# POSTECH-CVLab/RoDyGS

Measured on AMD Instinct MI355X. Metric: train-step fps at 1M dynamic Gaussians / 1080p (fwd+bwd+Adam, one camera per GPU per step), higher is better.
Workload: dtype f32; 1 GPU; 1000000 dynamic Gaussians + deformation MLP, 1920x1080, SH3, 100-frame synthetic video (BASELINE configs[2]); points=1000000, width=1920, height=1080, scene=uniform, frames=100, deferred_overflow_check=True, frame_order=orbit positions, bit-reversed, one_device=False, graph_replay=False, densify_stats=True, deterministic_backward=True, render_normal=True, parallelism=single GPU (frame-dp1), losses=photometric, sh_adam_in_backward=True, binning=bucket

## Files before the change

### rodygs_amd/csrc/rdg_render.hip

```cpp
#include "rdg_common.h"

#define RDG_BATCH 256

__device__ __forceinline__ int rdg_tile_of_block(int bid, int n_tiles) {
    const int per = (n_tiles + 7) >> 3;
    return (bid & 7) * per + (bid >> 3);
}

__device__ __forceinline__ float rdg_edge_min(float a, float b2, float c, float inv_c, float ue, float v0, float v1) {
    const float t = b2 * ue;
    const float vs = __builtin_amdgcn_fmed3f(-0.5f * t * inv_c, v0, v1);
    return fmaf(fmaf(c, vs, t), vs, a * ue * ue);
}
__device__ __forceinline__ uint32_t rdg_quadrant_bits(const float4 q0, const float4 q1, const float inv_cyy, float X0, float Y0) {
    const float a = q0.z, b = q0.w, o = q1.y;
    const float c = (b * b) / a + inv_cyy;
    const float t255 = 255.0f * o;
    if (!(t255 >= 0.99f)) return 0u;
    const float det = a * c - b * b;
    if (!(det > 0.0f) || !(a > 0.0f) || !(c > 0.0f)) return 0u;
    const float r2 = 2.0f * (__logf(t255) + 0.02f) * 1.001f;
    const float inv_a = 1.0f / a, inv_c = 1.0f / c, b2 = 2.0f * b;
    uint32_t bits = 0u;
#pragma unroll
    for (int qy = 0; qy < 2; ++qy) {
        const float v1 = q0.y - (Y0 + 8.0f * qy), v0 = v1 - 7.0f;
#pragma unroll
        for (int qx = 0; qx < 2; ++qx) {
            const float u1 = q0.x - (X0 + 8.0f * qx), u0 = u1 - 7.0f;
            const bool inside = u0 <= 0.0f && u1 >= 0.0f && v0 <= 0.0f && v1 >= 0.0f;
            const float m = fminf(fminf(rdg_edge_min(a, b2, c, inv_c, u0, v0, v1), rdg_edge_min(a, b2, c, inv_c, u1, v0, v1)),
                                  fminf(rdg_edge_min(c, b2, a, inv_a, v0, u0, u1), rdg_edge_min(c, b2, a, inv_a, v1, u0, u1)));
            bits |= (uint32_t)(inside || !(m > r2)) << (qy * 2 + qx);
        }
    }
    return bits;
}

#define RDG_NEG_LOG2E (-1.4426950408889634f)
struct RdgConicS { float hA, beta, gam; };
__device__ __forceinline__ RdgConicS rdg_stage_conic(float a, float b, float inv_cyy) {
    const float A2 = RDG_NEG_LOG2E * a, B = RDG_NEG_LOG2E * b;
    RdgConicS s;
    s.hA = 0.5f * A2;
    s.beta = (A2 < 0.0f) ? B / A2 : 0.0f;
    s.gam = (0.5f * RDG_NEG_LOG2E) * inv_cyy;
    return s;
}
__device__ __forceinline__ float rdg_log2_gauss(float hA, float beta, float gam, float dx, float dy) {
    const float w = fmaf(beta, dy, dx);
    return fmaf(hA * w, w, (gam * dy) * dy);
}
__device__ __forceinline__ float rdg_log2_gauss_w(float hA, float beta, float gam, float dx, float dy, float& w) {
    w = fmaf(beta, dy, dx);
    return fmaf(hA * w, w, (gam * dy) * dy);
}

__device__ __forceinline__ bool rdg_any(bool p) { return __builtin_amdgcn_ballot_w64(p) != 0ull; }
__device__ __forceinline__ bool rdg_all(bool p) { return __builtin_amdgcn_ballot_w64(!p) == 0ull; }

__device__ __forceinline__ unsigned long long rdg_uniform_u64(unsigned long long v) {
    const uint32_t lo = __builtin_amdgcn_readfirstlane((uint32_t)v);
    const uint32_t hi = __builtin_amdgcn_readfirstlane((uint32_t)(v >> 32));
    return ((unsigned long long)hi << 32) | lo;
}

#define RDG_THR_LIVE (0x80000000u | 0x3b808081u)
#define RDG_THR_DONE 0xffffffffu
template <bool NORMAL, bool CAPPED>
__device__ __forceinline__ void rdg_fwd_walk(unsigned long long mask, const unsigned long long cap, const int sbase,
                                             const uint32_t wbase, const char* sQ0, const char* sQ1, const char* sQ2,
                                             const char* sQ3, const float pixx, const float pixy,
                                             unsigned long long& seen, uint32_t& thrU, float& T,
                                             uint32_t& last_contributor, float& C0, float& C1, float& C2, float& Dp,
                                             float& N0, float& N1, float& N2) {
    while (mask) {
        const int jb = __builtin_ctzll(mask);
        asm("s_bitset0_b64 %0, %1" : "+s"(mask) : "s"(jb));
        int aj = (jb << 4) + sbase;
        asm volatile("" : "+v"(aj));
#ifdef RDG_ABL_FXSALU
        asm volatile("s_add_u32 s90, s90, 1\n\ts_add_u32 s91, s91, 1\n\ts_add_u32 s90, s90, 1\n\ts_add_u32 s91, s91, 1\n\t"
                     "s_add_u32 s90, s90, 1\n\ts_add_u32 s91, s91, 1\n\ts_add_u32 s90, s90, 1\n\ts_add_u32 s91, s91, 1" ::: "s90", "s91", "scc");
#endif
#ifdef RDG_ABL_FXVALU
        { float xa = T, xb = C0;
          asm volatile("v_mov_b32 %0, %1\n\tv_mov_b32 %1, %0\n\tv_mov_b32 %0, %1\n\tv_mov_b32 %1, %0\n\t"
                       "v_mov_b32 %0, %1\n\tv_mov_b32 %1, %0\n\tv_mov_b32 %0, %1\n\tv_mov_b32 %1, %0" : "+v"(xa), "+v"(xb)); }
#endif
        const float4 q0 = *(const float4*)(sQ0 + aj);
        const float2 q1 = *(const float2*)(sQ1 + aj);
        const float dx = q0.x - pixx, dy = q0.y - pixy;
        const float power = rdg_log2_gauss(q0.z, q0.w, q1.x, dx, dy);
        float alpha = q1.y * __builtin_amdgcn_exp2f(power);
        if (CAPPED && ((cap >> jb) & 1ull)) {
            asm volatile("; opacity above the cap" ::: "memory");
            alpha = fminf(RDG_ALPHA_CAP, alpha);
        }
        const uint32_t key = (__float_as_uint(power) & 0x80000000u) | __float_as_uint(alpha);
        const unsigned long long cand = __builtin_amdgcn_ballot_w64(key >= thrU);
        if (!cand) continue;
        asm("s_bitset1_b64 %0, %1" : "+s"(seen) : "s"(jb));
        float aeff;
        asm("v_cndmask_b32_e64 %0, 0, %1, %2" : "=v"(aeff) : "v"(alpha), "s"(cand));
        float test_T = T * (1.0f - aeff);
        float wgt = aeff * T;
        const float4 q2 = *(const float4*)(sQ2 + aj);
        const uint32_t idx = wbase + (uint32_t)jb;
        unsigned long long upd = cand;
        const unsigned long long stopm = __builtin_amdgcn_ballot_w64(test_T < RDG_T_STOP);
        if (stopm) {
            const bool stop = test_T < RDG_T_STOP;
            upd &= ~stopm;
            wgt = stop ? 0.0f : wgt;
            test_T = stop ? T : test_T;
            thrU = stop ? RDG_THR_DONE : thrU;
            if (rdg_all(thrU == RDG_THR_DONE)) { mask = 0ull; }
        }
        T = test_T;
        asm volatile("s_mov_b64 exec, %1\n\tv_mov_b32 %0, %2\n\ts_mov_b64 exec, -1"
                     : "+v"(last_contributor) : "s"(upd), "s"(idx));
        C0 += wgt * q2.x; C1 += wgt * q2.y; C2 += wgt * q2.z;
        Dp += wgt * q2.w;
        if (NORMAL) {
            const float4 q3 = *(const float4*)(sQ3 + aj);
            N0 += wgt * q3.x; N1 += wgt * q3.y; N2 += wgt * q3.z;
        }
    }
}


template <bool NORMAL>
__device__ __forceinline__ void
rdg_fwd_composite(const int k_begin, const int k_end, const uint2 range, const float X0, const float Y0, const float pixx,
                  const float pixy, const uint32_t* __restrict__ point_list, const RdgRec* __restrict__ rec,
                  unsigned long long* __restrict__ hit, float4* sQ0, float4* sQ1, float4* sQ2, float4* sQ3,
                  unsigned long long (*sMask)[4], unsigned long long* sCap, uint32_t& thrU, float& T, float& C0, float& C1,
                  float& C2, float& Dp, float& N0, float& N1, float& N2, uint32_t& last_contributor) {
    const int tid = threadIdx.x;
    const int lane = tid & 63, wv = tid >> 6;
    const int rounds = (k_end - k_begin + RDG_BATCH - 1) / RDG_BATCH;
    for (int r = 0; r < rounds; ++r) {
        if (__syncthreads_count(thrU == RDG_THR_DONE) == 256) break;
        const int k = k_begin + r * RDG_BATCH + tid;
        uint32_t qbits = 0;
        bool over_cap = false;
        if (k < k_end) {
            const uint32_t id = point_list[range.x + k];
            const RdgRec* p = rec + id;
            const float4 q0 = p->q0, q1 = p->q1, q2 = p->q2;
            const RdgConicS cs = rdg_stage_conic(q0.z, q0.w, q2.w);
            sQ0[tid] = make_float4(q0.x, q0.y, cs.hA, cs.beta);
            *(float2*)&sQ1[tid] = make_float2(cs.gam, q1.y);
            sQ2[tid] = make_float4(q2.x, q2.y, q2.z, q1.z);
            if (NORMAL) sQ3[tid] = p->q3;
            qbits = rdg_quadrant_bits(q0, q1, q2.w, X0, Y0);
            over_cap = q1.y > RDG_ALPHA_CAP;
        }
#pragma unroll
        for (int q = 0; q < 4; ++q) {
            const unsigned long long m = __ballot((qbits >> q) & 1u);
            if (lane == 0) sMask[q][wv] = m;
        }
        {
            const unsigned long long m = __ballot(over_cap);
            if (lane == 0) sCap[wv] = m;
        }
        __syncthreads();
#pragma unroll 1
        for (int s = 0; s < 4; ++s) {
            if (rdg_all(thrU == RDG_THR_DONE)) break;
            const unsigned long long mask = rdg_uniform_u64(sMask[wv][s]);
            const unsigned long long cap = rdg_uniform_u64(sCap[s]);
            unsigned long long seen = 0ull;
            const uint32_t wbase = (uint32_t)(k_begin + r * RDG_BATCH + s * 64 + 1);
            if (cap)
                rdg_fwd_walk<NORMAL, true>(mask, cap, s * 1024, wbase, (const char*)sQ0, (const char*)sQ1, (const char*)sQ2,
                                           (const char*)sQ3, pixx, pixy, seen, thrU, T, last_contributor, C0, C1, C2, Dp,
                                           N0, N1, N2);
            else
                rdg_fwd_walk<NORMAL, false>(mask, cap, s * 1024, wbase, (const char*)sQ0, (const char*)sQ1, (const char*)sQ2,
                                            (const char*)sQ3, pixx, pixy, seen, thrU, T, last_contributor, C0, C1, C2, Dp,
                                            N0, N1, N2);
            if (lane == 0 && seen) hit[(size_t)((k_begin >> 6) + r * 4 + s) * 4 + wv] = seen;
        }
    }
}

template <bool NORMAL>
__global__ void __launch_bounds__(256)
rdg_render_fwd_kernel(int W, int H, int gx, int n_tiles, const float* __restrict__ bg,
                      const uint2* __restrict__ ranges, const uint32_t* __restrict__ point_list,
                      const RdgRec* __restrict__ rec, long long capacity, const int32_t* __restrict__ num_rendered,
                      float* __restrict__ final_T, uint32_t* __restrict__ n_contrib, float* __restrict__ out_color,
                      float* __restrict__ out_depth, float* __restrict__ out_normal, float* __restrict__ out_alpha,
                      unsigned long long* __restrict__ hitbits, int split_min, uint4* __restrict__ zero_buf,
                      long long zero_n16) {
    if (zero_buf) {
        const long long per = (zero_n16 + gridDim.x - 1) / gridDim.x;
        const long long z0 = per * blockIdx.x, z1 = z0 + per < zero_n16 ? z0 + per : zero_n16;
        for (long long i = z0 + threadIdx.x; i < z1; i += 256) zero_buf[i] = make_uint4(0u, 0u, 0u, 0u);
    }
    const int tile = rdg_tile_of_block(blockIdx.x, n_tiles);
    if (tile >= n_tiles) return;
    __shared__ float4 sQ0[RDG_BATCH], sQ1[RDG_BATCH], sQ2[RDG_BATCH], sQ3[RDG_BATCH];
    __shared__ unsigned long long sMask[4][4];
    __shared__ unsigned long long sCap[4];
#ifdef RDG_ABL_FPAD
    __shared__ float sPad[RDG_ABL_FPAD];
    if (W < 0) sPad[threadIdx.x] = 1.0f;
#endif
    const int tid = threadIdx.x;
    const int lane = tid & 63, wv = tid >> 6;
    const int tx = tile % gx, ty = tile / gx;
    const int pxi = tx * RDG_TILE + (wv & 1) * 8 + (lane & 7);
    const int pyi = ty * RDG_TILE + (wv >> 1) * 8 + (lane >> 3);
    const bool inside = pxi < W && pyi < H;
    float pixx = (float)pxi, pixy = (float)pyi;
    asm volatile("" : "+v"(pixx), "+v"(pixy));
    const float X0 = (float)(tx * RDG_TILE), Y0 = (float)(ty * RDG_TILE);
    const uint2 range = ranges[tile];
    const int todo_total = (int)(range.y - range.x);
    if (todo_total > split_min) return;
    unsigned long long* const hit = hitbits + ((size_t)(range.x >> 6) + (size_t)tile) * 4;

    uint32_t thrU = inside ? RDG_THR_LIVE : RDG_THR_DONE;
    float T = 1.0f;
    float C0 = 0.f, C1 = 0.f, C2 = 0.f, Dp = 0.f, N0 = 0.f, N1 = 0.f, N2 = 0.f;
    uint32_t last_contributor = 0;
    rdg_fwd_composite<NORMAL>(0, todo_total, range, X0, Y0, pixx, pixy, point_list, rec, hit, sQ0, sQ1, sQ2, sQ3, sMask,
                              sCap, thrU, T, C0, C1, C2, Dp, N0, N1, N2, last_contributor);
    if (inside) {
        const size_t hw = (size_t)H * W;
        const size_t pid = (size_t)pyi * W + pxi;
        final_T[pid] = T;
        n_contrib[pid] = last_contributor;
        out_color[pid] = C0 + T * bg[0];
        out_color[hw + pid] = C1 + T * bg[1];
        out_color[2 * hw + pid] = C2 + T * bg[2];
        out_depth[pid] = Dp;
        out_alpha[pid] = 1.0f - T;
        out_normal[pid] = N0; out_normal[hw + pid] = N1; out_normal[2 * hw + pid] = N2;
    }
}

#define RDG_SEG_TS 0
#define RDG_SEG_TOUT 1
#define RDG_SEG_C 2
#define RDG_SEG_LAST 9
#define RDG_SEG_LIVE 10

__device__ __forceinline__ float* rdg_seg_row(float* seg_pix, uint32_t seg, int field) {
    return seg_pix + ((size_t)seg * RDG_SEG_F + field) * RDG_TILE_PIX;
}

__global__ void __launch_bounds__(256)
rdg_render_seg_T_kernel(int W, int H, int gx, const uint2* __restrict__ ranges, const uint32_t* __restrict__ point_list,
                        const RdgRec* __restrict__ rec, const uint32_t* __restrict__ sp_header,
                        const uint4* __restrict__ sp_work, float* __restrict__ seg_pix) {
    __shared__ float4 sQ0[RDG_BATCH];
    __shared__ float2 sQ1[RDG_BATCH];
    const int tid = threadIdx.x;
    const uint32_t n_work = sp_header[0];
    for (uint32_t wi = blockIdx.x; wi < n_work; wi += gridDim.x) {
        const uint4 w = sp_work[wi];
        const int tile = (int)w.x;
        const int tx = tile % gx, ty = tile / gx;
        const int wv = tid >> 6, lane = tid & 63;
        const int pxi = tx * RDG_TILE + (wv & 1) * 8 + (lane & 7);
        const int pyi = ty * RDG_TILE + (wv >> 1) * 8 + (lane >> 3);
        const float pixx = (float)pxi, pixy = (float)pyi;
        const uint2 range = ranges[tile];
        const int k_begin = (int)w.y * RDG_SPLIT_SEG, k_end = min(k_begin + RDG_SPLIT_SEG, (int)(range.y - range.x));
        float T = 1.0f;
        for (int k0 = k_begin; k0 < k_end; k0 += RDG_BATCH) {
            __syncthreads();
            const int k = k0 + tid;
            if (k < k_end) {
                const RdgRec* p = rec + point_list[range.x + k];
                const float4 q0 = p->q0, q1 = p->q1;
                const RdgConicS cs = rdg_stage_conic(q0.z, q0.w, p->q2.w);
                sQ0[tid] = make_float4(q0.x, q0.y, cs.hA, cs.beta);
                sQ1[tid] = make_float2(cs.gam, q1.y);
            }
            __syncthreads();
            const int n = min(RDG_BATCH, k_end - k0);
            for (int j = 0; j < n; ++j) {
                const float4 q0 = sQ0[j];
                const float2 q1 = sQ1[j];
                const float dx = q0.x - pixx, dy = q0.y - pixy;
                const float power = rdg_log2_gauss(q0.z, q0.w, q1.x, dx, dy);
                float alpha = q1.y * __builtin_amdgcn_exp2f(power);
                if (q1.y > RDG_ALPHA_CAP) alpha = fminf(RDG_ALPHA_CAP, alpha);
                const uint32_t key = (__float_as_uint(power) & 0x80000000u) | __float_as_uint(alpha);
                if (key >= RDG_THR_LIVE) T = T * (1.0f - alpha);
            }
        }
        rdg_seg_row(seg_pix, w.w + w.y, RDG_SEG_TS)[tid] = T;
    }
}

template <bool NORMAL>
__global__ void __launch_bounds__(256)
rdg_render_seg_kernel(int W, int H, int gx, const uint2* __restrict__ ranges, const uint32_t* __restrict__ point_list,
                      const RdgRec* __restrict__ rec, const uint32_t* __restrict__ sp_header,
                      const uint4* __restrict__ sp_work, float* __restrict__ seg_pix,
                      unsigned long long* __restrict__ hitbits) {
    __shared__ float4 sQ0[RDG_BATCH], sQ1[RDG_BATCH], sQ2[RDG_BATCH], sQ3[RDG_BATCH];
    __shared__ unsigned long long sMask[4][4];
    __shared__ unsigned long long sCap[4];
    const int tid = threadIdx.x;
    const int lane = tid & 63, wv = tid >> 6;
    const uint32_t n_work = sp_header[0];
    for (uint32_t wi = blockIdx.x; wi < n_work; wi += gridDim.x) {
// ... 54 lines not shown
        float T = 1.0f, C0 = 0.f, C1 = 0.f, C2 = 0.f, Dp = 0.f, N0 = 0.f, N1 = 0.f, N2 = 0.f;
        uint32_t last = 0;
        for (uint32_t s = 0; s < t.y; ++s) {
            const float* base = seg_pix + (size_t)(t.z + s) * RDG_SEG_F * RDG_TILE_PIX + tid;
            if (base[RDG_SEG_LIVE * RDG_TILE_PIX] == 0.0f) continue;
            T = base[RDG_SEG_TOUT * RDG_TILE_PIX];
            C0 += base[(RDG_SEG_C + 0) * RDG_TILE_PIX]; C1 += base[(RDG_SEG_C + 1) * RDG_TILE_PIX];
            C2 += base[(RDG_SEG_C + 2) * RDG_TILE_PIX]; Dp += base[(RDG_SEG_C + 3) * RDG_TILE_PIX];
            if (NORMAL) {
                N0 += base[(RDG_SEG_C + 4) * RDG_TILE_PIX]; N1 += base[(RDG_SEG_C + 5) * RDG_TILE_PIX];
                N2 += base[(RDG_SEG_C + 6) * RDG_TILE_PIX];
            }
            last = max(last, __float_as_uint(base[RDG_SEG_LAST * RDG_TILE_PIX]));
        }
        const size_t hw = (size_t)H * W;
        const size_t pid = (size_t)pyi * W + pxi;
        final_T[pid] = T;
        n_contrib[pid] = last;
        out_color[pid] = C0 + T * bg[0];
        out_color[hw + pid] = C1 + T * bg[1];
        out_color[2 * hw + pid] = C2 + T * bg[2];
        out_depth[pid] = Dp;
        out_alpha[pid] = 1.0f - T;
        out_normal[pid] = N0; out_normal[hw + pid] = N1; out_normal[2 * hw + pid] = N2;
    }
}

__global__ void __launch_bounds__(1024)
rdg_split_build_kernel(int n_tiles, const uint2* __restrict__ ranges, long long capacity,
                       const int32_t* __restrict__ num_rendered, uint32_t* __restrict__ sp_header,
                       uint4* __restrict__ sp_work, uint4* __restrict__ sp_tiles, uint32_t max_seg, uint32_t max_tiles) {
    __shared__ uint32_t sSeg, sTiles;
    if (threadIdx.x == 0) { sSeg = 0u; sTiles = 0u; }
    __syncthreads();
    if ((long long)num_rendered[0] <= capacity)
        for (int i = threadIdx.x; i < n_tiles; i += 1024) {
            const uint2 r = ranges[i];
            const uint32_t n = r.y - r.x;
            if (n > (uint32_t)RDG_SPLIT_MIN) {
                const uint32_t nseg = (n + RDG_SPLIT_SEG - 1) / RDG_SPLIT_SEG;
                const uint32_t base = atomicAdd(&sSeg, nseg), ti = atomicAdd(&sTiles, 1u);
                if (base + nseg <= max_seg && ti < max_tiles) {
                    sp_tiles[ti] = make_uint4((uint32_t)i, nseg, base, 0u);
                    for (uint32_t c = 0; c < nseg; ++c) sp_work[base + c] = make_uint4((uint32_t)i, c, nseg, base);
                }
            }
        }
    __syncthreads();
    if (threadIdx.x == 0) { sp_header[0] = min(sSeg, max_seg); sp_header[1] = min(sTiles, max_tiles); }
}

int rdg_launch_split_build(const RdgDev& d, void* bin_ws, int64_t capacity, const void* image_ws,
                           const int32_t* num_rendered, hipStream_t s) {
    const int n_tiles = d.gx * d.gy;
    const RdgBinLayout B = rdg_bin_layout(capacity, n_tiles);
    const RdgSplitLayout SL = rdg_split_layout(capacity);
    const RdgImageLayout I = rdg_image_layout(d.H, d.W);
    char* sp = (char*)bin_ws + B.split;
    hipLaunchKernelGGL(rdg_split_build_kernel, dim3(1), dim3(1024), 0, s, n_tiles,
                       (const uint2*)((const char*)image_ws + I.ranges), (long long)capacity, num_rendered,
                       (uint32_t*)(sp + SL.header), (uint4*)(sp + SL.work), (uint4*)(sp + SL.tiles), SL.max_seg,
                       SL.max_tiles);
    return rdg_check_hip(hipGetLastError(), "split_build launch");
}

int rdg_launch_render_fwd(const RdgDev& d, const float* bg, const void* geom_ws, void* bin_ws,
                          int64_t capacity, void* image_ws, const int32_t* num_rendered, float* out_color,
                          float* out_depth, float* out_normal, float* out_alpha, hipStream_t s) {
    const RdgGeomLayout G = rdg_geom_layout(d.P);
    const int n_tiles = d.gx * d.gy;
    const RdgBinLayout B = rdg_bin_layout(capacity, n_tiles);
    const RdgImageLayout I = rdg_image_layout(d.H, d.W);
    const int npass = (rdg_key_bits(n_tiles) + RDG_SORT_BITS - 1) / RDG_SORT_BITS;
    const char* b = (const char*)bin_ws;
    const uint32_t* plist = (const uint32_t*)(b + ((npass & 1) ? B.vals_b : B.vals_a));
    char* im = (char*)image_ws;
    const int nblk = ((n_tiles + 7) / 8) * 8;
    const RdgRec* rec = (const RdgRec*)((const char*)geom_ws + G.rec);
    const uint2* ranges = (const uint2*)(im + I.ranges);
    float* final_T = (float*)(im + I.final_T);
    uint32_t* n_contrib = (uint32_t*)(im + I.n_contrib);
    unsigned long long* hitbits = (unsigned long long*)((char*)bin_ws + B.hit);
    const int split_min = (d.list_hints & 1) ? RDG_SPLIT_MIN : 0x7fffffff;
#define RDG_FWD_LAUNCH(NORMAL)                                                                                      \
    hipLaunchKernelGGL(rdg_render_fwd_kernel<NORMAL>, dim3(nblk), dim3(256), 0, s, d.W, d.H, d.gx, n_tiles, bg,       \
                       ranges, plist, rec, (long long)capacity, num_rendered, final_T, n_contrib,                    \
                       out_color, out_depth, out_normal, out_alpha, hitbits, split_min, (uint4*)d.zero_grad_ws,     \
                       zero_n16)
    const long long zero_n16 = (long long)(rdg_align_up((size_t)(d.P > 0 ? d.P : 1) * RDG_GROW * 4, 256) / 16);
    if (d.render_normal) RDG_FWD_LAUNCH(true); else RDG_FWD_LAUNCH(false);
#undef RDG_FWD_LAUNCH
    if ((d.list_hints & 1)) {
        int rc = rdg_launch_split_build(d, bin_ws, capacity, image_ws, num_rendered, s);
        if (rc) return rc;
        const RdgSplitLayout SL = rdg_split_layout(capacity);
        char* sp = (char*)bin_ws + B.split;
        const uint32_t* sp_header = (const uint32_t*)(sp + SL.header);
        const uint4* sp_work = (const uint4*)(sp + SL.work);
        const uint4* sp_tiles = (const uint4*)(sp + SL.tiles);
        float* seg_pix = (float*)(sp + SL.seg_pix);
        const unsigned gseg = SL.max_seg < 2048u ? SL.max_seg : 2048u, gtile = SL.max_tiles < 1024u ? SL.max_tiles : 1024u;
        hipLaunchKernelGGL(rdg_render_seg_T_kernel, dim3(gseg), dim3(256), 0, s, d.W, d.H, d.gx, ranges, plist, rec,
                           sp_header, sp_work, seg_pix);
        if (d.render_normal) {
            hipLaunchKernelGGL(rdg_render_seg_kernel<true>, dim3(gseg), dim3(256), 0, s, d.W, d.H, d.gx, ranges, plist, rec,
                               sp_header, sp_work, seg_pix, hitbits);
            hipLaunchKernelGGL(rdg_render_seg_combine_kernel<true>, dim3(gtile), dim3(256), 0, s, d.W, d.H, d.gx, bg,
                               sp_header, sp_tiles, (const float*)seg_pix, final_T, n_contrib, out_color, out_depth,
                               out_normal, out_alpha);
        } else {
            hipLaunchKernelGGL(rdg_render_seg_kernel<false>, dim3(gseg), dim3(256), 0, s, d.W, d.H, d.gx, ranges, plist, rec,
                               sp_header, sp_work, seg_pix, hitbits);
            hipLaunchKernelGGL(rdg_render_seg_combine_kernel<false>, dim3(gtile), dim3(256), 0, s, d.W, d.H, d.gx, bg,
                               sp_header, sp_tiles, (const float*)seg_pix, final_T, n_contrib, out_color, out_depth,
                               out_normal, out_alpha);
        }
    }
    return rdg_check_hip(hipGetLastError(), "render_fwd launch");
}

#ifndef RDG_RING
#define RDG_RING 4
#endif
#define RDG_RING_Q 6
template <bool HAS_DEPTH, bool DET>
__device__ __forceinline__ void rdg_ring_flush(float (*ring)[16][RDG_RING_Q], int n, int lane, float scale, int foff,
                                               float* __restrict__ grow) {
    __builtin_amdgcn_fence(__ATOMIC_RELEASE, "wavefront");
    __builtin_amdgcn_wave_barrier();
    __builtin_amdgcn_fence(__ATOMIC_ACQUIRE, "wavefront");
    const int c = lane & 15;
    for (int e0 = 0; e0 < n; e0 += 4) {
        const int e = e0 + (lane >> 4);
        if (e < n && c < (HAS_DEPTH ? 10 : 9)) {
            const float* r = &ring[e][0][0] + foff;
            constexpr int G = 2 * RDG_RING_Q;
            const float v = (((r[0] + r[G]) + (r[2 * G] + r[3 * G])) + ((r[4 * G] + r[5 * G]) + (r[6 * G] + r[7 * G]))) * scale;
#ifdef RDG_ABL_NOATOMIC
            if (v == 123.456f) atomicAdd(grow + (size_t)__float_as_uint(ring[e][1][4]) * RDG_GROW + c, v);
#else
            if (DET) grow[(size_t)__float_as_uint(ring[e][1][4]) * (4 * RDG_GROW) + c] = v;
            else if (v != 0.0f) atomicAdd(grow + (size_t)__float_as_uint(ring[e][1][4]) * RDG_GROW + c, v);
#endif
        }
    }
    __builtin_amdgcn_fence(__ATOMIC_RELEASE, "wavefront");
    __builtin_amdgcn_wave_barrier();
    __builtin_amdgcn_fence(__ATOMIC_ACQUIRE, "wavefront");
}

template <bool HAS_DEPTH, bool CAPPED, bool DET, bool ALLBELOW, bool HAS_NORMAL>
__device__ __forceinline__ void rdg_bwd_walk(unsigned long long mask, const unsigned long long cap, const int sbase,
                                             const char* sQ0, const char* sQ1, const char* sQ2, const char* sQ3,
                                             const float pixx, const float pixy, const int jthr, const float dLp0,
                                             const float dLp1, const float dLp2, const float dLd, const float dLn0,
                                             const float dLn1, const float dLn2, const int lane,
                                             float (*ring)[16][RDG_RING_Q], const float flush_scale, const int flush_off,
                                             float* __restrict__ grow, float& T, float& behind, int& ring_n) {
    while (mask) {
        const int jb = __builtin_ctzll(mask);
        asm("s_bitset0_b64 %0, %1" : "+s"(mask) : "s"(jb));
        int aj = (jb << 4) + sbase;
        asm volatile("" : "+v"(aj));
        const float4 q0 = *(const float4*)(sQ0 + aj);
        const float4 q1 = *(const float4*)(sQ1 + aj);
        const float dx = q0.x - pixx, dy = q0.y - pixy;
        float wsk;
        const float power = rdg_log2_gauss_w(q0.z, q0.w, q1.x, dx, dy, wsk);
        const float G = __builtin_amdgcn_exp2f(power);
        float alpha = q1.y * G;
        const bool capped = CAPPED && ((cap >> jb) & 1ull);
        if (capped) {
            asm volatile("; opacity above the cap" ::: "memory");
// ... 369 lines not shown
```

### rodygs_amd/rasterizer.py

```python
from __future__ import annotations

import ctypes as C
import os
import threading
from typing import NamedTuple, Optional

import torch
import torch.nn as nn

from . import _lib

RENDER_NORMAL = True
PREZERO_GRAD_ROWS = os.environ.get("RDG_PREZERO_GRAD_ROWS", "1") != "0"
NREN_HOST_MIRROR = os.environ.get("RDG_NREN_MIRROR", "1") != "0"
BIN_RADIX_ABOVE = 32768
BIN_BUCKET_BELOW = 16384
BIN_RADIX_MEAN_LIST_ABOVE = 1000
BIN_BUCKET_MEAN_LIST_BELOW = 800
SPLIT_ABOVE = 4096
SPLIT_BELOW = 3072
_FORCE_RADIX = os.environ.get("RDG_BIN_MODE", "") == "radix"
_FORCE_BUCKET = os.environ.get("RDG_BIN_MODE", "") == "bucket"

DETERMINISTIC = os.environ.get("RDG_DETERMINISTIC", "0") == "1"

CULL = os.environ.get("RDG_CULL", "1") != "0"

GRAPH_CAPTURE = False

HINT_DECAY = 0.98
DEFERRED_OVERFLOW_CHECK = False


class RasterizerCapacityOverflow(RuntimeError):
    """Raised (deferred mode only) when an earlier forward produced more (tile, Gaussian) instances than its binning
    workspace could hold.  That frame was rendered as an EMPTY scene (background, zero gradients); the capacity hint
    has been raised, so re-running the frame succeeds."""


class RasterState:

    def __init__(self, deterministic: Optional[bool] = None, force_radix: Optional[bool] = None,
                 force_bucket: Optional[bool] = None, deferred_overflow_check: Optional[bool] = None,
                 render_normal: Optional[bool] = None, cull: Optional[bool] = None):
        self.deterministic, self.force_radix, self.force_bucket = deterministic, force_radix, force_bucket
        self.deferred_overflow_check, self.render_normal = deferred_overflow_check, render_normal
        self.cull = cull
        self.capacity_hint = {}
        self.d_high = {}
        self.bin_hint = {}
        self.split_hint = {}
        self.pending = []
        self.pinned_free = []
        self.last_nren = None
        self.last_image = None
        self.graph_capture = False
        self.nren_max = None
        self.nren_max_key = None
        self.det_ws = None
        self.aux_stream = None
        self.pose_grad = None
        self.pose_fork_eager = None
        self.keep_alive = []
        self.lock = threading.RLock()

    def mode(self, name: str) -> bool:
        v = getattr(self, name)
        if v is not None:
            return bool(v)
        return bool({"deterministic": DETERMINISTIC, "force_radix": _FORCE_RADIX, "force_bucket": _FORCE_BUCKET,
                     "deferred_overflow_check": DEFERRED_OVERFLOW_CHECK, "render_normal": RENDER_NORMAL,
                     "cull": CULL}[name])

    def note_instances(self, key, n: int) -> None:
        self.d_high[key] = max(int(n), int(self.d_high.get(key, 0) * HINT_DECAY))

    def pinned_slot(self) -> torch.Tensor:
        return self.pinned_free.pop() if self.pinned_free else torch.empty(2, dtype=torch.int32).pin_memory()

    def note_largest_tile(self, key, largest: int, n: int = 0) -> None:
        tiles = ((key[2] + 15) // 16) * ((key[1] + 15) // 16)
        mean = n / max(tiles, 1)
        if (largest > BIN_RADIX_ABOVE or mean > BIN_RADIX_MEAN_LIST_ABOVE) and not self.mode("force_bucket"):
            self.bin_hint[key] = 1
        elif largest < BIN_BUCKET_BELOW and mean < BIN_BUCKET_MEAN_LIST_BELOW:
            self.bin_hint.pop(key, None)
        if largest > SPLIT_ABOVE:
            self.split_hint[key] = 1
        elif largest < SPLIT_BELOW:
            self.split_hint.pop(key, None)

    def poll_overflow(self, block: bool = False) -> None:
        with self.lock:
            while self.pending:
                stream, host, key, cap, nren = self.pending[0]
                if int(host[0]) < 0:
                    if not block:
                        return
                    stream.synchronize()
                    if int(host[0]) < 0:
                        host[0], host[1] = (int(v) for v in nren.tolist())
                n = int(host[0])
                self.pending.pop(0)
                self.pinned_free.append(host)
                if n >= _INSTANCE_LIMIT:
                    raise RuntimeError(_too_many(key))
                self.capacity_hint[key] = max(n, int(self.capacity_hint.get(key, 0) * HINT_DECAY))
                self.note_instances(key, n)
                self.note_largest_tile(key, int(host[1]), n)
# ... 115 lines not shown
    rows = sink.get("rows")
    for k, t in arrs.items():
        if t is None:
            continue
        if not t.is_cuda or t.dtype != torch.float32 or not t.is_contiguous():
            raise RuntimeError(f"grad_sinks['densify']['{k}'] must be a contiguous float32 GPU tensor")
        rows = t.numel() if rows is None else rows
        if t.numel() != rows:
            raise RuntimeError("grad_sinks['densify']: the statistics arrays must all hold `rows` elements")
    if rows is None:
        return
    rows = int(rows)
    if row0 < 0 or row0 + rows > P:
        raise RuntimeError(f"grad_sinks['densify']: rows [{row0}, {row0 + rows}) do not lie inside the {P} Gaussians")
    cs.densify_grad_accum = _lib.ptr(arrs["grad_accum"])
    cs.densify_denom = _lib.ptr(arrs["denom"])
    cs.densify_max_radii = _lib.ptr(arrs["max_radii"])
    cs.densify_row0, cs.densify_rows = row0, rows


class _RasterizeGaussians(torch.autograd.Function):
    @staticmethod
    def forward(ctx, means3D, means2D, sh, colors_precomp, opacities, scales, rotations, cov3Ds_precomp, viewmatrix,
                raster_settings, grad_sinks=None, state=None):
        L = _lib.lib()
        ctx.grad_sinks = grad_sinks
        state = state if state is not None else DEFAULT_STATE
        ctx.state = state
        dev = means3D.device
        sh, colors_precomp = _empty(sh), _empty(colors_precomp)
        scales, rotations, cov3Ds_precomp = _empty(scales), _empty(rotations), _empty(cov3Ds_precomp)
        m3 = _f32c(means3D, "means3D", dev)
        shs = _f32c(sh, "shs", dev)
        col = _f32c(colors_precomp, "colors_precomp", dev)
        op = _f32c(opacities, "opacities", dev)
        sc = _f32c(scales, "scales", dev)
        ro = _f32c(rotations, "rotations", dev)
        cov = _f32c(cov3Ds_precomp, "cov3Ds_precomp", dev)
        vm = _f32c(viewmatrix, "viewmatrix", dev)
        pm = _f32c(raster_settings.projmatrix, "projmatrix", dev)
        bg = _f32c(raster_settings.bg, "bg", dev)
        P = m3.shape[0]
        if m3.dim() != 2 or m3.shape[1] != 3:
            raise RuntimeError("means3D must be [P,3]")
        if op.numel() != P:
            raise RuntimeError("opacities must be [P,1]")
        if vm.numel() != 16 or pm.numel() != 16 or bg.numel() != 3:
            raise RuntimeError("viewmatrix/projmatrix must be [4,4] and bg [3]")
        M = 0
        if shs is not None:
            if shs.dim() != 3 or shs.shape[0] != P or shs.shape[2] != 3:
                raise RuntimeError("shs must be [P,K,3]")
            M = shs.shape[1]
        if P == 0:
            ph = torch.zeros(16, 3, dtype=torch.float32, device=dev)
            shs, col, cov, sc, ro, M = ph, None, None, ph, ph, 16
            op = ph if op.numel() == 0 else op
            m3 = ph
        H, W = int(raster_settings.image_height), int(raster_settings.image_width)
        cs = _c_settings(raster_settings, P, M, state)
        n_tiles = ((W + 15) // 16) * ((H + 15) // 16)
        ctx.deterministic = det_mode = state.mode("deterministic")

        with torch.cuda.device(dev):
            u8 = dict(dtype=torch.uint8, device=dev)
            geom = torch.empty(L.rdg_geom_bytes(P), **u8)
            image = torch.empty(L.rdg_image_bytes(H, W), **u8)
            color = torch.empty(3, H, W, dtype=torch.float32, device=dev)
            depth = torch.empty(1, H, W, dtype=torch.float32, device=dev)
            normal = torch.empty(3, H, W, dtype=torch.float32, device=dev)
            alpha = torch.empty(1, H, W, dtype=torch.float32, device=dev)
            radii = torch.empty(P, dtype=torch.int32, device=dev)
            gws = None
            if PREZERO_GRAD_ROWS and P > 0 and not det_mode and any(ctx.needs_input_grad):
                gws = torch.empty(L.rdg_grad_bytes(P), **u8)
                cs.zero_grad_ws = gws.data_ptr()
            nren = torch.empty(2, dtype=torch.int32, device=dev)
            key = (P, H, W)
            cs.num_rendered_stats = 1
            capture = GRAPH_CAPTURE or state.graph_capture
            stream = _lib.stream_ptr()
            with state.lock:
                cs.bin_mode = max(int(cs.bin_mode), int(state.bin_hint.get(key, 0)))
                cs.list_hints = 1 if det_mode else int(state.split_hint.get(key, 0))
                cap = max(int(state.capacity_hint.get(key, 0) * 1.25) + 4096, 4 * P + 4096)
                if capture and key not in state.capacity_hint:
                    raise RuntimeError("graph capture needs a warm-up forward of this (P, H, W) on the same RasterState first")
                deferred = state.mode("deferred_overflow_check") and key in state.capacity_hint and not capture
                if deferred:
                    state.poll_overflow(block=False)
                host = None
                if deferred:
                    host = state.pinned_slot()
                    host[0], host[1] = -1, -1
                    if NREN_HOST_MIRROR:
                        cs.num_rendered_host = host.data_ptr()
                if state.nren_max is not None and state.nren_max_key in (None, key):
                    cs.num_rendered_max = state.nren_max.data_ptr()
            while True:
                binning = torch.empty(L.rdg_binning_bytes(cap, n_tiles), **u8)
                rc = L.rdg_rasterize_forward(C.byref(cs), _lib.ptr(bg), _lib.ptr(m3), _lib.ptr(shs), _lib.ptr(col),
                                             _lib.ptr(op), _lib.ptr(sc), _lib.ptr(ro), _lib.ptr(cov), _lib.ptr(vm),
                                             _lib.ptr(pm), _lib.ptr(geom), _lib.ptr(binning), cap, _lib.ptr(image),
                                             _lib.ptr(color), _lib.ptr(depth), _lib.ptr(normal), _lib.ptr(alpha),
                                             _lib.ptr(radii), _lib.ptr(nren), stream)
                _lib.check(rc, "rdg_rasterize_forward")
                state.last_nren = (nren, key, cap)
                if capture:
                    n = -1
                    break
                if deferred:
                    if not NREN_HOST_MIRROR:
                        host.copy_(nren, non_blocking=True)
                    with state.lock:
                        state.pending.append((torch.cuda.current_stream(dev), host, key, cap, nren))
                    n = -1
                    break
                n, largest = (int(v) for v in nren.tolist())
                if n >= _INSTANCE_LIMIT:
                    raise RuntimeError(_too_many(key))
                with state.lock:
                    checked = (state.nren_max is not None and state.nren_max_key in (None, key)) or bool(state.pending)
                    state.capacity_hint[key] = max(n, int(state.capacity_hint.get(key, 0) * HINT_DECAY)) if checked else n
                    state.note_instances(key, n)
                    state.note_largest_tile(key, largest, n)
                if n <= cap:
                    break
                cap = int(n * 1.25) + 4096
        state.last_image = (image, H, W)
        ctx.set_materialize_grads(False)
        ctx.raster_settings = raster_settings
        ctx.empty_cloud = (P == 0)
        ctx.cs = cs
        ctx.gws = gws
        ctx.capacity = cap
        ctx.num_rendered = n
        ctx.has = (shs is not None, col is not None, sc is not None, cov is not None)
        ctx.save_for_backward(m3, shs, col, op, sc, ro, cov, vm, pm, bg, radii, geom, binning, image)
        extra = torch.empty(0, dtype=torch.float32, device=dev)
        ctx.mark_non_differentiable(radii, extra)
        return color, depth, normal, alpha, radii, extra

    @staticmethod
    def backward(ctx, g_color, g_depth, g_normal, g_alpha, g_radii, g_extra):
        if g_normal is not None and not ctx.cs.render_normal:
            raise RuntimeError("rodygs_amd rasterizer: rendered_normal received an upstream gradient, but the forward ran "
                               "with rasterizer.RENDER_NORMAL = False (the image is all zeros and has no graph)")
        if ctx.empty_cloud or (g_color is None and g_depth is None and g_alpha is None and g_normal is None):
            return (None,) * 12
        L = _lib.lib()
        m3, shs, col, op, sc, ro, cov, vm, pm, bg, radii, geom, binning, image = ctx.saved_tensors
        dev = m3.device
        P = m3.shape[0]
        f32 = dict(dtype=torch.float32, device=dev)

        def gc(t):
            return None if t is None else t.to(torch.float32).contiguous()

        g_color, g_depth, g_alpha, g_normal = gc(g_color), gc(g_depth), gc(g_alpha), gc(g_normal)
        with torch.cuda.device(dev):
            gws, ctx.gws = ctx.gws, None
            _bind_densify_stats(ctx, P)
            ctx.cs.grad_rows_zeroed = 1 if (gws is not None and not ctx.deterministic) else 0
            if gws is None:
                gws = torch.empty(L.rdg_grad_bytes(P), dtype=torch.uint8, device=dev)
            d_m3 = torch.empty(P, 3, **f32)
            d_m2 = torch.empty(P, 3, **f32)
# ... 156 lines not shown
```

Measured before the change: 723.5 frames/s.

## Add row-compacted forward walk with 4x4 sub-block culling per wave

Adds a new forward rasterization path that tests each Gaussian against sixteen 4x4 pixel sub-blocks using exact ellipse row extents. Per wave it builds compacted per-row index lists in shared memory, so each 16-lane row group walks only the Gaussians that touch its 4x4 block. Pixels are remapped so lane groups line up with these sub-blocks. This path is the default and replaces the old quadrant-mask walk, which stays reachable through an environment flag. The kernel also requests 8 waves per EU. The aim is fewer wasted alpha evaluations, paid for with extra ballots, list construction, shared memory and register pressure.

```diff
diff --git a/rodygs_amd/csrc/rdg_render.hip b/rodygs_amd/csrc/rdg_render.hip
--- a/rodygs_amd/csrc/rdg_render.hip
+++ b/rodygs_amd/csrc/rdg_render.hip
@@ -32,6 +32,35 @@
             const float m = fminf(fminf(rdg_edge_min(a, b2, c, inv_c, u0, v0, v1), rdg_edge_min(a, b2, c, inv_c, u1, v0, v1)),
                                   fminf(rdg_edge_min(c, b2, a, inv_a, v0, u0, u1), rdg_edge_min(c, b2, a, inv_a, v1, u0, u1)));
             bits |= (uint32_t)(inside || !(m > r2)) << (qy * 2 + qx);
+        }
+    }
+    return bits;
+}
+__device__ __forceinline__ uint32_t rdg_block_bits(const float4 q0, const float4 q1, const float inv_cyy, float X0, float Y0) {
+    const float a = q0.z, b = q0.w, o = q1.y;
+    const float c = (b * b) / a + inv_cyy;
+    const float t255 = 255.0f * o;
+    if (!(t255 >= 0.99f)) return 0u;
+    const float det = a * c - b * b;
+    if (!(det > 0.0f) || !(a > 0.0f) || !(c > 0.0f)) return 0u;
+    const float r2 = 2.0f * (__logf(t255) + 0.02f) * 1.001f;
+    const float inv_a = 1.0f / a, r2a = r2 * a;
+    const float ys = b * __builtin_amdgcn_sqrtf(r2 / (c * det));
+    const float ye = __builtin_amdgcn_sqrtf(r2a / det);
+    uint32_t bits = 0u;
+#pragma unroll
+    for (int by = 0; by < 4; ++by) {
+        const float y0 = (Y0 + 4.0f * by) - q0.y;
+        const float lo = fmaxf(y0, -ye), hi = fminf(y0 + 3.0f, ye);
+        if (lo > hi) continue;
+        const float yA = __builtin_amdgcn_fmed3f(-ys, lo, hi), yB = __builtin_amdgcn_fmed3f(ys, lo, hi);
+        const float xmax = (__builtin_amdgcn_sqrtf(fmaxf(fmaf(-det * yA, yA, r2a), 0.0f)) - b * yA) * inv_a;
+        const float xmin = (-__builtin_amdgcn_sqrtf(fmaxf(fmaf(-det * yB, yB, r2a), 0.0f)) - b * yB) * inv_a;
+#pragma unroll
+        for (int bx = 0; bx < 4; ++bx) {
+            const float x0 = (X0 + 4.0f * bx) - q0.x;
+            const int bit = ((by >> 1) * 2 + (bx >> 1)) * 4 + (by & 1) * 2 + (bx & 1);
+            bits |= (uint32_t)(!(xmin > x0 + 3.0f) && !(xmax < x0)) << bit;
         }
     }
     return bits;
@@ -187,8 +216,141 @@
     }
 }
 
+#define RDG_ROW_SENT (RDG_BATCH * 16)
+#define RDG_ROW_LIST 65
+template <bool NORMAL, bool CAPPED>
+__device__ __forceinline__ void rdg_fwd_row_walk(int n, int la, const uint32_t wb1, const uint32_t fbase, const char* sL,
+                                                 const char* sQ0, const char* sQ1, const char* sQ2, const char* sQ3,
+                                                 const float pixx, const float pixy, uint32_t& thrU, float& T,
+                                                 uint32_t& last_contributor, float& C0, float& C1, float& C2, float& Dp,
+                                                 float& N0, float& N1, float& N2) {
+    int nxt = *(const unsigned short*)(sL + la);
+    for (int i = 0; i < n; ++i) {
+        const int aj = nxt;
+        la += 8;
+        asm volatile("" : "+v"(la));
+        nxt = *(const unsigned short*)(sL + la);
+        const float4 q0 = *(const float4*)(sQ0 + aj);
+        const float2 q1 = *(const float2*)(sQ1 + aj);
+        const float dx = q0.x - pixx, dy = q0.y - pixy;
+        const float power = rdg_log2_gauss(q0.z, q0.w, q1.x, dx, dy);
+        float alpha = q1.y * __builtin_amdgcn_exp2f(power);
+        if (CAPPED) alpha = q1.y > RDG_ALPHA_CAP ? fminf(RDG_ALPHA_CAP, alpha) : alpha;
+        const uint32_t key = (__float_as_uint(power) & 0x80000000u) | __float_as_uint(alpha);
+        const unsigned long long cand = __builtin_amdgcn_ballot_w64(key >= thrU);
+        if (!cand) continue;
+        {
+            const uint32_t fa = fbase + (uint32_t)aj;
+            asm volatile("s_mov_b64 exec, %1\n\tds_write_b8 %0, %0\n\ts_mov_b64 exec, -1" : : "v"(fa), "s"(cand) : "memory");
+        }
+        float aeff;
+        asm("v_cndmask_b32_e64 %0, 0, %1, %2" : "=v"(aeff) : "v"(alpha), "s"(cand));
+        float test_T = T * (1.0f - aeff);
+        float wgt = aeff * T;
+        const float4 q2 = *(const float4*)(sQ2 + aj);
+        unsigned long long upd = cand;
+        const unsigned long long stopm = __builtin_amdgcn_ballot_w64(test_T < RDG_T_STOP);
+        if (stopm) {
+            const bool stop = test_T < RDG_T_STOP;
+            upd &= ~stopm;
+            wgt = stop ? 0.0f : wgt;
+            test_T = stop ? T : test_T;
+            thrU = stop ? RDG_THR_DONE : thrU;
+            if (rdg_all(thrU == RDG_THR_DONE)) { n = 0; }
+        }
+        T = test_T;
+        asm volatile("s_mov_b64 exec, %1\n\tv_lshrrev_b32 %0, 4, %3\n\tv_add_u32 %0, %2, %0\n\ts_mov_b64 exec, -1"
+                     : "+v"(last_contributor) : "s"(upd), "s"(wb1), "v"(aj));
+        C0 += wgt * q2.x; C1 += wgt * q2.y; C2 += wgt * q2.z;
+        Dp += wgt * q2.w;
+        if (NORMAL) {
+            const float4 q3 = *(const float4*)(sQ3 + aj);
+            N0 += wgt * q3.x; N1 += wgt * q3.y; N2 += wgt * q3.z;
+        }
+    }
+}
+
 template <bool NORMAL>
-__global__ void __launch_bounds__(256)
+__device__ __forceinline__ void
+rdg_fwd_composite_rows(const int k_end, const uint2 range, const float X0, const float Y0, const float pixx,
+                       const float pixy, const uint32_t* __restrict__ point_list, const RdgRec* __restrict__ rec,
+                       unsigned long long* __restrict__ hit, float4* sQ0, float4* sQ1, float4* sQ2, float4* sQ3,
+                       unsigned long long (*sBlk)[4], unsigned long long* sCap, unsigned short* sList, uint32_t& thrU,
+                       float& T, float& C0, float& C1, float& C2, float& Dp, float& N0, float& N1, float& N2,
+                       uint32_t& last_contributor) {
+    const int tid = threadIdx.x;
+    const int lane = tid & 63, wv = tid >> 6;
+    unsigned short (*const L)[4] = (unsigned short (*)[4])(sList + wv * RDG_ROW_LIST * 4);
+    const int la0 = (int)((wv * RDG_ROW_LIST * 4 + (lane >> 4)) * 2);
+    const uint32_t fbase = (uint32_t)(size_t)sQ1 + 8u + (uint32_t)wv;
+    const int rounds = (k_end + RDG_BATCH - 1) / RDG_BATCH;
+    for (int r = 0; r < rounds; ++r) {
+        if (__syncthreads_count(thrU == RDG_THR_DONE) == 256) break;
+        const int k = r * RDG_BATCH + tid;
+        uint32_t bbits = 0;
+        bool over_cap = false;
+        float4 s1 = make_float4(0.f, 0.f, 0.f, 0.f);
+        if (k < k_end) {
+            const uint32_t id = point_list[range.x + k];
+            const RdgRec* p = rec + id;
+            const float4 q0 = p->q0, q1 = p->q1, q2 = p->q2;
+            const RdgConicS cs = rdg_stage_conic(q0.z, q0.w, q2.w);
+            sQ0[tid] = make_float4(q0.x, q0.y, cs.hA, cs.beta);
+            s1.x = cs.gam; s1.y = q1.y;
+            sQ2[tid] = make_float4(q2.x, q2.y, q2.z, q1.z);
+            if (NORMAL) sQ3[tid] = p->q3;
+            bbits = rdg_block_bits(q0, q1, q2.w, X0, Y0);
+            over_cap = q1.y > RDG_ALPHA_CAP;
+        }
+        sQ1[tid] = s1;
+#pragma unroll
+        for (int b = 0; b < 16; ++b) {
+            const unsigned long long m = __ballot((bbits >> b) & 1u);
+            if (lane == 0) sBlk[b][wv] = m;
+        }
+        {
+            const unsigned long long m = __ballot(over_cap);
+            if (lane == 0) sCap[wv] = m;
+        }
+        __syncthreads();
+#pragma unroll 1
+        for (int s = 0; s < 4; ++s) {
+            if (rdg_all(thrU == RDG_THR_DONE)) break;
+            const unsigned long long m0 = rdg_uniform_u64(sBlk[wv * 4 + 0][s]), m1 = rdg_uniform_u64(sBlk[wv * 4 + 1][s]);
+            const unsigned long long m2 = rdg_uniform_u64(sBlk[wv * 4 + 2][s]), m3 = rdg_uniform_u64(sBlk[wv * 4 + 3][s]);
+            const int n = max(max(__popcll(m0), __popcll(m1)), max(__popcll(m2), __popcll(m3)));
+            if (n == 0) continue;
+            *(unsigned long long*)&L[lane][0] = 0x1000100010001000ull;
+            const unsigned short off = (unsigned short)((s * 64 + lane) * 16);
+#define RDG_ROW_PUT(M, R)                                                                                              \
+            if (((M) >> lane) & 1ull)                                                                                  \
+                L[__builtin_amdgcn_mbcnt_hi((uint32_t)((M) >> 32), __builtin_amdgcn_mbcnt_lo((uint32_t)(M), 0u))][R] = off
+            RDG_ROW_PUT(m0, 0); RDG_ROW_PUT(m1, 1); RDG_ROW_PUT(m2, 2); RDG_ROW_PUT(m3, 3);
+#undef RDG_ROW_PUT
+            __builtin_amdgcn_fence(__ATOMIC_RELEASE, "wavefront");
+            __builtin_amdgcn_wave_barrier();
+            __builtin_amdgcn_fence(__ATOMIC_ACQUIRE, "wavefront");
+            const unsigned long long cap = rdg_uniform_u64(sCap[s]);
+            const uint32_t wb1 = (uint32_t)(r * RDG_BATCH + 1);
+            if (cap)
+                rdg_fwd_row_walk<NORMAL, true>(n, la0, wb1, fbase, (const char*)sList, (const char*)sQ0, (const char*)sQ1,
+                                               (const char*)sQ2, (const char*)sQ3, pixx, pixy, thrU, T, last_contributor,
+                                               C0, C1, C2, Dp, N0, N1, N2);
+            else
+                rdg_fwd_row_walk<NORMAL, false>(n, la0, wb1, fbase, (const char*)sList, (const char*)sQ0, (const char*)sQ1,
+                                                (const char*)sQ2, (const char*)sQ3, pixx, pixy, thrU, T, last_contributor,
+                                                C0, C1, C2, Dp, N0, N1, N2);
+            __builtin_amdgcn_fence(__ATOMIC_RELEASE, "wavefront");
+            __builtin_amdgcn_wave_barrier();
+            __builtin_amdgcn_fence(__ATOMIC_ACQUIRE, "wavefront");
+            const unsigned long long seen = __ballot(((const unsigned char*)sQ1)[(s * 64 + lane) * 16 + 8 + wv] != 0);
+            if (lane == 0 && seen) hit[(size_t)(r * 4 + s) * 4 + wv] = seen;
+        }
+    }
+}
+
+template <bool NORMAL, bool ROWS>
+__global__ void __launch_bounds__(256) __attribute__((amdgpu_waves_per_eu(8)))
 rdg_render_fwd_kernel(int W, int H, int gx, int n_tiles, const float* __restrict__ bg,
                       const uint2* __restrict__ ranges, const uint32_t* __restrict__ point_list,
                       const RdgRec* __restrict__ rec, long long capacity, const int32_t* __restrict__ num_rendered,
@@ -203,9 +365,10 @@
     }
     const int tile = rdg_tile_of_block(blockIdx.x, n_tiles);
     if (tile >= n_tiles) return;
-    __shared__ float4 sQ0[RDG_BATCH], sQ1[RDG_BATCH], sQ2[RDG_BATCH], sQ3[RDG_BATCH];
-    __shared__ unsigned long long sMask[4][4];
+    __shared__ float4 sQ0[RDG_BATCH + ROWS], sQ1[RDG_BATCH + ROWS], sQ2[RDG_BATCH + ROWS], sQ3[RDG_BATCH + ROWS];
+    __shared__ unsigned long long sMask[ROWS ? 16 : 4][4];
     __shared__ unsigned long long sCap[4];
+    __shared__ unsigned short sList[ROWS ? 4 * RDG_ROW_LIST * 4 : 1];
 #ifdef RDG_ABL_FPAD
     __shared__ float sPad[RDG_ABL_FPAD];
     if (W < 0) sPad[threadIdx.x] = 1.0f;
@@ -213,8 +376,8 @@
     const int tid = threadIdx.x;
     const int lane = tid & 63, wv = tid >> 6;
     const int tx = tile % gx, ty = tile / gx;
-    const int pxi = tx * RDG_TILE + (wv & 1) * 8 + (lane & 7);
-    const int pyi = ty * RDG_TILE + (wv >> 1) * 8 + (lane >> 3);
+    const int pxi = tx * RDG_TILE + (wv & 1) * 8 + (ROWS ? ((lane >> 4) & 1) * 4 + (lane & 3) : (lane & 7));
+    const int pyi = ty * RDG_TILE + (wv >> 1) * 8 + (ROWS ? (lane >> 5) * 4 + ((lane >> 2) & 3) : (lane >> 3));
     const bool inside = pxi < W && pyi < H;
     float pixx = (float)pxi, pixy = (float)pyi;
     asm volatile("" : "+v"(pixx), "+v"(pixy));
@@ -228,8 +391,17 @@
     float T = 1.0f;
     float C0 = 0.f, C1 = 0.f, C2 = 0.f, Dp = 0.f, N0 = 0.f, N1 = 0.f, N2 = 0.f;
     uint32_t last_contributor = 0;
-    rdg_fwd_composite<NORMAL>(0, todo_total, range, X0, Y0, pixx, pixy, point_list, rec, hit, sQ0, sQ1, sQ2, sQ3, sMask,
-                              sCap, thrU, T, C0, C1, C2, Dp, N0, N1, N2, last_contributor);
+    if (ROWS) {
+        if (tid == 0) {
+            sQ0[RDG_BATCH] = make_float4(0.f, 0.f, 0.f, 0.f); sQ1[RDG_BATCH] = make_float4(0.f, 0.f, 0.f, 0.f);
+            sQ2[RDG_BATCH] = make_float4(0.f, 0.f, 0.f, 0.f); sQ3[RDG_BATCH] = make_float4(0.f, 0.f, 0.f, 0.f);
+        }
+        rdg_fwd_composite_rows<NORMAL>(todo_total, range, X0, Y0, pixx, pixy, point_list, rec, hit, sQ0, sQ1, sQ2, sQ3,
+                                       sMask, sCap, sList, thrU, T, C0, C1, C2, Dp, N0, N1, N2, last_contributor);
+    } else {
+        rdg_fwd_composite<NORMAL>(0, todo_total, range, X0, Y0, pixx, pixy, point_list, rec, hit, sQ0, sQ1, sQ2, sQ3,
+                                  sMask, sCap, thrU, T, C0, C1, C2, Dp, N0, N1, N2, last_contributor);
+    }
     if (inside) {
         const size_t hw = (size_t)H * W;
         const size_t pid = (size_t)pyi * W + pxi;
@@ -450,13 +622,15 @@
     uint32_t* n_contrib = (uint32_t*)(im + I.n_contrib);
     unsigned long long* hitbits = (unsigned long long*)((char*)bin_ws + B.hit);
     const int split_min = (d.list_hints & 1) ? RDG_SPLIT_MIN : 0x7fffffff;
-#define RDG_FWD_LAUNCH(NORMAL)                                                                                      \
-    hipLaunchKernelGGL(rdg_render_fwd_kernel<NORMAL>, dim3(nblk), dim3(256), 0, s, d.W, d.H, d.gx, n_tiles, bg,       \
+    const bool rows = !(d.list_hints & 2);
+#define RDG_FWD_LAUNCH(NORMAL, ROWS)                                                                                \
+    hipLaunchKernelGGL((rdg_render_fwd_kernel<NORMAL, ROWS>), dim3(nblk), dim3(256), 0, s, d.W, d.H, d.gx, n_tiles, bg, \
                        ranges, plist, rec, (long long)capacity, num_rendered, final_T, n_contrib,                    \
                        out_color, out_depth, out_normal, out_alpha, hitbits, split_min, (uint4*)d.zero_grad_ws,     \
                        zero_n16)
     const long long zero_n16 = (long long)(rdg_align_up((size_t)(d.P > 0 ? d.P : 1) * RDG_GROW * 4, 256) / 16);
-    if (d.render_normal) RDG_FWD_LAUNCH(true); else RDG_FWD_LAUNCH(false);
+    if (d.render_normal) { if (rows) RDG_FWD_LAUNCH(true, true); else RDG_FWD_LAUNCH(true, false); }
+    else { if (rows) RDG_FWD_LAUNCH(false, true); else RDG_FWD_LAUNCH(false, false); }
 #undef RDG_FWD_LAUNCH
     if ((d.list_hints & 1)) {
         int rc = rdg_launch_split_build(d, bin_ws, capacity, image_ws, num_rendered, s);
diff --git a/rodygs_amd/rasterizer.py b/rodygs_amd/rasterizer.py
--- a/rodygs_amd/rasterizer.py
+++ b/rodygs_amd/rasterizer.py
@@ -25,6 +25,7 @@
 DETERMINISTIC = os.environ.get("RDG_DETERMINISTIC", "0") == "1"
 
 CULL = os.environ.get("RDG_CULL", "1") != "0"
+QUADRANT_WALK = os.environ.get("RDG_QUADRANT_WALK", "0") == "1"
 
 GRAPH_CAPTURE = False
 
@@ -306,7 +307,7 @@
             stream = _lib.stream_ptr()
             with state.lock:
                 cs.bin_mode = max(int(cs.bin_mode), int(state.bin_hint.get(key, 0)))
-                cs.list_hints = 1 if det_mode else int(state.split_hint.get(key, 0))
+                cs.list_hints = (1 if det_mode else int(state.split_hint.get(key, 0))) | (2 if QUADRANT_WALK else 0)
                 cap = max(int(state.capacity_hint.get(key, 0) * 1.25) + 4096, 4 * P + 4096)
                 if capture and key not in state.capacity_hint:
                     raise RuntimeError("graph capture needs a warm-up forward of this (P, H, W) on the same RasterState first")
```

Result: no change. 723.0 frames/s, median of 4 (-0.1%).
